# evenrose/CMDIAD

Measured on NVIDIA B200. Metric: patch-NN scores/sec at 200k x 768 bank, higher is better.
Workload: dtype f32 (fp16 tensor-core pre-filter with an error-bound certificate, exact fp32 re-check, FP32-equivalent fp16 hi/lo fallback)

## Files before the change

cmdiad_b200/csrc/score_gemm.cu:

```cuda
#include <cuda.h>

#include <cstdlib>

#include "common.cuh"

namespace cmdb {

constexpr int BM = kScoreBM;
constexpr int BN = kScoreBN;
constexpr int BK = kScoreBK;
constexpr int UMMA_K = 16;
constexpr int kGemmCtlThreads = 128;
constexpr uint32_t kTileABytes = BM * BK * 2;
constexpr uint32_t kTileBBytes = BN * BK * 2;
constexpr uint32_t kTmemCols = 512;

template <int TERMS, int CG>
struct GemmSmem {
    static constexpr uint32_t kTileB = kTileBBytes / CG;
    static constexpr int kStages = (TERMS == 3 ? 2 : 4) * (CG == 2 ? 3 : 2) / 2;
    static constexpr uint32_t kStageBytes = (TERMS == 3 ? 2u : 1u) * (kTileABytes + kTileB);
    static constexpr uint32_t stage(int s) { return s * kStageBytes; }
    static constexpr uint32_t a_hi(int s) { return stage(s); }
    static constexpr uint32_t b_hi(int s) { return stage(s) + kTileABytes; }
// ... 101 lines not shown
__device__ __forceinline__ void tc_fence_before() { asm volatile("tcgen05.fence::before_thread_sync;" ::: "memory"); }
__device__ __forceinline__ void tc_fence_after() { asm volatile("tcgen05.fence::after_thread_sync;" ::: "memory"); }
__device__ __forceinline__ void tmem_ld32(uint32_t taddr, uint32_t (&r)[32]) {
    asm volatile(
        "tcgen05.ld.sync.aligned.32x32b.x32.b32 "
        "{%0,%1,%2,%3,%4,%5,%6,%7,%8,%9,%10,%11,%12,%13,%14,%15,%16,%17,%18,%19,%20,%21,%22,%23,%24,%25,%26,%27,%28,%29,%30,%31}, "
        "[%32];"
        : "=r"(r[0]), "=r"(r[1]), "=r"(r[2]), "=r"(r[3]), "=r"(r[4]), "=r"(r[5]), "=r"(r[6]), "=r"(r[7]), "=r"(r[8]),
          "=r"(r[9]), "=r"(r[10]), "=r"(r[11]), "=r"(r[12]), "=r"(r[13]), "=r"(r[14]), "=r"(r[15]), "=r"(r[16]),
          "=r"(r[17]), "=r"(r[18]), "=r"(r[19]), "=r"(r[20]), "=r"(r[21]), "=r"(r[22]), "=r"(r[23]), "=r"(r[24]),
          "=r"(r[25]), "=r"(r[26]), "=r"(r[27]), "=r"(r[28]), "=r"(r[29]), "=r"(r[30]), "=r"(r[31])
        : "r"(taddr)
        : "memory");
}
__device__ __forceinline__ void tmem_ld_wait() { asm volatile("tcgen05.wait::ld.sync.aligned;" ::: "memory"); }

__device__ __forceinline__ uint64_t make_sw128_desc(uint32_t smem_addr) {
    uint64_t d = 0;
    d |= (uint64_t)((smem_addr & 0x3FFFFu) >> 4);
    d |= (uint64_t)((8u * BK * 2u) >> 4) << 32;
    d |= (uint64_t)1 << 46;
    d |= (uint64_t)2 << 61;
    return d;
}
constexpr uint32_t kIdesc = (1u << 4) | ((uint32_t)(BN >> 3) << 17) | ((uint32_t)(BM >> 4) << 24);
constexpr uint32_t kIdescPair = (1u << 4) | ((uint32_t)(BN >> 3) << 17) | ((uint32_t)((2 * BM) >> 4) << 24);

__device__ __forceinline__ int tile_stride(int mt, int G) {
    for (int s = mt;; ++s) {
        int a = s % G, b = G;
        if (a == 0) a = G;
        while (b) {
            const int t = a % b;
            a = b, b = t;
        }
        if (a == 1 || G == 1) return s;
    }
}
struct TileIter {
    int n, m, base, smod, G;
    __device__ __forceinline__ TileIter(int c, int G_, int mt, int stride) {
        G = G_;
        smod = stride % G;
        n = -1, m = mt, base = (c + smod) % G;
    }
    __device__ __forceinline__ bool next(int mt, int nt) {
        m += G;
        while (m >= mt) {
            if (++n >= nt) return false;
            base -= smod;
            if (base < 0) base += G;
            m = base;
        }
        return true;
    }
};

struct Top2 {
    float b1, b2;
    int i1, i2;
};
__device__ __forceinline__ void top2_update(Top2 &t, float v, int col) {
    const bool c1 = v < t.b1, c2 = v < t.b2;
    t.i2 = c1 ? t.i1 : (c2 ? col : t.i2);
    t.b2 = fminf(t.b2, fmaxf(t.b1, v));
    t.i1 = c1 ? col : t.i1;
    t.b1 = fminf(t.b1, v);
}
__device__ __forceinline__ void top2_insert(Top2 &t, float v, int i) {
    if (i < 0) return;
    const bool c1 = t.i1 < 0 || v < t.b1 || (v == t.b1 && i < t.i1);
    const bool c2 = t.i2 < 0 || v < t.b2 || (v == t.b2 && i < t.i2);
    if (c1) t.b2 = t.b1, t.i2 = t.i1, t.b1 = v, t.i1 = i;
    else if (c2) t.b2 = v, t.i2 = i;
}
__device__ __forceinline__ void top2_chunk(const uint32_t (&r)[32], float c, const float *bn, int col, Top2 &ta, Top2 &tb) {
#pragma unroll
    for (int k = 0; k < 32; k += 2) {
        top2_update(ta, fmaf(__uint_as_float(r[k]), c, bn[k]), col + k);
        top2_update(tb, fmaf(__uint_as_float(r[k + 1]), c, bn[k + 1]), col + k + 1);
    }
}

struct GemmParams {
    int mt;
    int m_base;
    const int *m_count;
    int nt;
    int kb;
    const float *bnorm;
    const int *q_scale_exp;
    int b_scale_exp;
    float4 *cand;
    int cand_stride;
    int run;
};

template <int TERMS, int EG, int CG>
__global__ void __launch_bounds__(kGemmCtlThreads + 128 * EG, 1)
score_gemm_kernel(const __grid_constant__ CUtensorMap tm_qhi, const __grid_constant__ CUtensorMap tm_qlo,
                  const __grid_constant__ CUtensorMap tm_bhi, const __grid_constant__ CUtensorMap tm_blo, GemmParams p) {
    using S = GemmSmem<TERMS, CG>;
    constexpr int kGemmThreads = kGemmCtlThreads + 128 * EG;
    extern __shared__ __align__(1024) unsigned char smem_raw[];
    unsigned char *smem = smem_raw + ((1024u - (smem_u32(smem_raw) & 1023u)) & 1023u);
    const uint32_t sbase = smem_u32(smem);
    const int warp = threadIdx.x >> 5, lane = threadIdx.x & 31;
    if (p.m_count) {
        p.mt = (__ldg(p.m_count) + BM - 1) / BM;
        if (p.mt == 0) return;
    }
    const int rank = CG == 2 ? (int)cluster_ctarank() : 0;
    const int unit = (int)blockIdx.x / CG, n_units = (int)gridDim.x / CG;
    const int mt_units = (p.mt + CG - 1) / CG;
    const int stride = tile_stride(mt_units, n_units);
    const int nruns = (p.nt + p.run - 1) / p.run;
    const uint32_t bar_full = sbase + S::bars, bar_empty = bar_full + 8 * S::kStages;
    const uint32_t bar_tfull = bar_empty + 8 * S::kStages, bar_tempty = bar_tfull + 16;
    uint32_t *tmem_slot = reinterpret_cast<uint32_t *>(smem + S::bars + 8 * (2 * S::kStages + 4));
    float *bnorm_s = reinterpret_cast<float *>(smem + S::bnorm);
    float4 *state = p.cand + (size_t)blockIdx.x * EG * p.cand_stride;

    if (warp == 1 && lane == 0) {
        for (int s = 0; s < S::kStages; ++s) {
            mbar_init(bar_full + 8 * s, 1);
            mbar_init(bar_empty + 8 * s, 1);
        }
        for (int b = 0; b < 2; ++b) {
            mbar_init(bar_tfull + 8 * b, 1);
            mbar_init(bar_tempty + 8 * b, 4 * EG * CG);
        }
        asm volatile("fence.mbarrier_init.release.cluster;" ::: "memory");
    }
    if (warp == 2) {
        if constexpr (CG == 2) tmem_alloc_pair(smem_u32(tmem_slot), kTmemCols);
        else tmem_alloc(smem_u32(tmem_slot), kTmemCols);
    }
    for (int i = p.m_base * BM + threadIdx.x; i < (p.m_base + p.mt) * BM; i += kGemmThreads)
#pragma unroll
        for (int g = 0; g < EG; ++g)
            state[(size_t)g * p.cand_stride + i] = make_float4(INFINITY, __int_as_float(-1), INFINITY, __int_as_float(-1));
    __threadfence_block();
    tc_fence_before();
    __syncthreads();
    if constexpr (CG == 2) cluster_sync_all();
    tc_fence_after();
    const uint32_t tmem_base = *tmem_slot;

    if (warp == 0) {
        if (lane == 0) {
            int stage = 0;
            uint32_t phase = 0;
            for (TileIter it(unit, n_units, mt_units, stride); it.next(mt_units, nruns);) {
              const int m = it.m * CG + rank;
              for (int n = it.n * p.run, n_end = min(p.nt, n + p.run); n < n_end; ++n) {
                const int a_row = (p.m_base + m) * BM, b_row = n * BN + rank * (BN / CG);
                for (int kb = 0; kb < p.kb; ++kb) {
                    mbar_wait(bar_empty + 8 * stage, phase ^ 1);
                    if constexpr (CG == 2) {
                        const uint32_t full = map_to_cta(bar_full + 8 * stage, 0);
                        if (rank == 0) mbar_expect_tx(bar_full + 8 * stage, 2 * S::kStageBytes);
                        tma_load_2d_pair(sbase + S::a_hi(stage), &tm_qhi, full, kb * BK, a_row);
                        tma_load_2d_pair(sbase + S::b_hi(stage), &tm_bhi, full, kb * BK, b_row);
                        if constexpr (TERMS == 3) {
                            tma_load_2d_pair(sbase + S::a_lo(stage), &tm_qlo, full, kb * BK, a_row);
                            tma_load_2d_pair(sbase + S::b_lo(stage), &tm_blo, full, kb * BK, b_row);
                        }
                    } else {
                        const uint32_t full = bar_full + 8 * stage;
                        mbar_expect_tx(full, S::kStageBytes);
                        tma_load_2d(sbase + S::a_hi(stage), &tm_qhi, full, kb * BK, a_row);
                        tma_load_2d(sbase + S::b_hi(stage), &tm_bhi, full, kb * BK, b_row);
                        if constexpr (TERMS == 3) {
                            tma_load_2d(sbase + S::a_lo(stage), &tm_qlo, full, kb * BK, a_row);
                            tma_load_2d(sbase + S::b_lo(stage), &tm_blo, full, kb * BK, b_row);
                        }
                    }
                    if (++stage == S::kStages) stage = 0, phase ^= 1;
                }
              }
            }
        }
    } else if (warp == 1) {
        if (lane == 0 && rank == 0) {
            int stage = 0;
            uint32_t phase = 0;
            int j = 0;
            for (TileIter it(unit, n_units, mt_units, stride); it.next(mt_units, nruns);)
              for (int n = it.n * p.run, n_end = min(p.nt, n + p.run); n < n_end; ++n, ++j) {
                const int buf = j & 1;
                mbar_wait(bar_tempty + 8 * buf, ((j >> 1) & 1) ^ 1);
                tc_fence_after();
                const uint32_t tmem_d = tmem_base + buf * BN;
                for (int kb = 0; kb < p.kb; ++kb) {
                    mbar_wait(bar_full + 8 * stage, phase);
                    tc_fence_after();
                    const uint64_t a_hi = make_sw128_desc(sbase + S::a_hi(stage));
                    const uint64_t a_lo = make_sw128_desc(sbase + S::a_lo(stage));
                    const uint64_t b_hi = make_sw128_desc(sbase + S::b_hi(stage));
                    const uint64_t b_lo = make_sw128_desc(sbase + S::b_lo(stage));
#pragma unroll
                    for (int ks = 0; ks < BK / UMMA_K; ++ks) {
                        const uint64_t adv = (uint64_t)((ks * UMMA_K * 2) >> 4);
                        if constexpr (CG == 2) {
                            umma_f16_pair(tmem_d, a_hi + adv, b_hi + adv, kIdescPair, (kb | ks) != 0);
                            if constexpr (TERMS == 3) {
                                umma_f16_pair(tmem_d, a_hi + adv, b_lo + adv, kIdescPair, 1);
                                umma_f16_pair(tmem_d, a_lo + adv, b_hi + adv, kIdescPair, 1);
                            }
                        } else {
                            umma_f16(tmem_d, a_hi + adv, b_hi + adv, kIdesc, (kb | ks) != 0);
                            if constexpr (TERMS == 3) {
                                umma_f16(tmem_d, a_hi + adv, b_lo + adv, kIdesc, 1);
                                umma_f16(tmem_d, a_lo + adv, b_hi + adv, kIdesc, 1);
                            }
                        }
                    }
                    if constexpr (CG == 2) umma_commit_pair(bar_empty + 8 * stage);
                    else umma_commit(bar_empty + 8 * stage);
                    if (++stage == S::kStages) stage = 0, phase ^= 1;
                }
                if constexpr (CG == 2) umma_commit_pair(bar_tfull + 8 * buf);
                else umma_commit(bar_tfull + 8 * buf);
            }
        }
    } else if (warp >= 4) {
        const int quarter = warp & 3;
        const int half = (warp - 4) >> 2;
        const int row = quarter * 32 + lane;
        const int et = threadIdx.x - kGemmCtlThreads;
        constexpr int kHalfCols = BN / EG;
        float4 *my_state = state + (size_t)half * p.cand_stride;
        const uint32_t tempty_leader = CG == 2 ? map_to_cta(bar_tempty, 0) : bar_tempty;
        auto release_tmem = [&](int buf) {
            tc_fence_before();
            __syncwarp();
            if (lane == 0) {
                if constexpr (CG == 2) mbar_arrive_cluster(tempty_leader + 8 * buf);
                else mbar_arrive(bar_tempty + 8 * buf);
            }
        };
        int j = 0;
        for (TileIter it(unit, n_units, mt_units, stride); it.next(mt_units, nruns);) {
          const int m_tile = it.m * CG + rank;
          const bool valid = m_tile < p.mt;
          const int m_local = p.m_base + m_tile;
          float c = 0.f;
          Top2 ta{INFINITY, INFINITY, -1, -1};
          if (valid) {
              c = ldexpf(-2.f, -(p.b_scale_exp + __ldg(p.q_scale_exp + m_local * BM + row)));
              const float4 st = my_state[m_local * BM + row];
              ta = Top2{st.x, st.z, __float_as_int(st.y), __float_as_int(st.w)};
          }
          for (int n = it.n * p.run, n_end = min(p.nt, n + p.run); n < n_end; ++n, ++j) {
            const int buf = j & 1;
            float *bn = bnorm_s + buf * BN;
#pragma unroll
            for (int g = 0; g < 2 / EG; ++g) bn[et + g * 128 * EG] = __ldg(p.bnorm + (size_t)n * BN + et + g * 128 * EG);
            Top2 tb{INFINITY, INFINITY, -1, -1};
            mbar_wait(bar_tfull + 8 * buf, (j >> 1) & 1);
            tc_fence_after();
            asm volatile("bar.sync 1, %0;" ::"n"(128 * EG) : "memory");
            if (!valid) {
                release_tmem(buf);
                continue;
            }
            const uint32_t taddr = tmem_base + ((uint32_t)(quarter * 32) << 16) + buf * BN + half * kHalfCols;
            const int col0 = n * BN + half * kHalfCols;
            const float *bnh = bn + half * kHalfCols;
            uint32_t ra[32], rb[32];
            tmem_ld32(taddr, ra);
#pragma unroll 1
            for (int ch = 0; ch < kHalfCols / 32; ch += 2) {
                tmem_ld_wait();
                tmem_ld32(taddr + (ch + 1) * 32, rb);
                top2_chunk(ra, c, bnh + ch * 32, col0 + ch * 32, ta, tb);
                tmem_ld_wait();
                if (ch + 2 < kHalfCols / 32) tmem_ld32(taddr + (ch + 2) * 32, ra);
                else release_tmem(buf);
                top2_chunk(rb, c, bnh + (ch + 1) * 32, col0 + (ch + 1) * 32, ta, tb);
            }
            top2_insert(ta, tb.b1, tb.i1);
            top2_insert(ta, tb.b2, tb.i2);
          }
          if (valid) my_state[m_local * BM + row] = make_float4(ta.b1, __int_as_float(ta.i1), ta.b2, __int_as_float(ta.i2));
        }
    }
    tc_fence_before();
    __syncthreads();
    if constexpr (CG == 2) cluster_sync_all();
    if (warp == 2) {
        tc_fence_after();
        if constexpr (CG == 2) tmem_dealloc_pair(tmem_base, kTmemCols);
        else tmem_dealloc(tmem_base, kTmemCols);
    }
}

__global__ void __launch_bounds__(256) q_split_kernel(const float *__restrict__ q, int P, int P_pad, int dim,
                                                      __half *__restrict__ hi, __half *__restrict__ lo,
                                                      int *__restrict__ scale_exp_out, float *__restrict__ q_norm,
                                                      float *__restrict__ q_eps, const int *__restrict__ list,
                                                      const int *__restrict__ count) {
    const int lane = threadIdx.x & 31, dim4 = dim >> 2;
    if (count) {
        P = __ldg(count);
        P_pad = (P + BM - 1) / BM * BM;
    }
    for (int r = blockIdx.x * 8 + (threadIdx.x >> 5); r < P_pad; r += gridDim.x * 8) {
        uint2 *h = reinterpret_cast<uint2 *>(hi + (size_t)r * dim), *l = reinterpret_cast<uint2 *>(lo + (size_t)r * dim);
        const float *src = q + (size_t)((list && r < P) ? __ldg(list + r) : r) * dim;
        float amax = 0.f;
        if (r < P)
            for (int cc = lane; cc < dim4; cc += 32) {
                const float4 v = __ldg(reinterpret_cast<const float4 *>(src) + cc);
                amax = fmaxf(fmaxf(amax, fmaxf(fabsf(v.x), fabsf(v.y))), fmaxf(fabsf(v.z), fabsf(v.w)));
            }
#pragma unroll
        for (int o = 16; o > 0; o >>= 1) amax = fmaxf(amax, __shfl_xor_sync(0xffffffffu, amax, o));
        int e = 0;
        if (amax > 0.f && amax < INFINITY) {
            int ex;
            frexpf(amax, &ex);
            e = 13 - ex;
        }
        if (lane == 0) scale_exp_out[r] = e;
        const float scale = ldexpf(1.f, e);
        float n2 = 0.f, e2 = 0.f;
        for (int cc = lane; cc < dim4; cc += 32) {
            float4 v = make_float4(0.f, 0.f, 0.f, 0.f);
            if (r < P) v = __ldg(reinterpret_cast<const float4 *>(src) + cc);
            v.x *= scale, v.y *= scale, v.z *= scale, v.w *= scale;
            __half2 h0 = __floats2half2_rn(v.x, v.y), h1 = __floats2half2_rn(v.z, v.w);
            const float2 f0 = __half22float2(h0), f1 = __half22float2(h1);
            const float r0 = v.x - f0.x, r1 = v.y - f0.y, r2 = v.z - f1.x, r3 = v.w - f1.y;
            n2 = fmaf(v.x, v.x, fmaf(v.y, v.y, fmaf(v.z, v.z, fmaf(v.w, v.w, n2))));
            e2 = fmaf(r0, r0, fmaf(r1, r1, fmaf(r2, r2, fmaf(r3, r3, e2))));
            __half2 l0 = __floats2half2_rn(r0, r1), l1 = __floats2half2_rn(r2, r3);
            h[cc] = make_uint2(*reinterpret_cast<unsigned int *>(&h0), *reinterpret_cast<unsigned int *>(&h1));
            l[cc] = make_uint2(*reinterpret_cast<unsigned int *>(&l0), *reinterpret_cast<unsigned int *>(&l1));
        }
        if (q_norm) {
#pragma unroll
            for (int o = 16; o > 0; o >>= 1) {
                n2 += __shfl_xor_sync(0xffffffffu, n2, o);
                e2 += __shfl_xor_sync(0xffffffffu, e2, o);
            }
            if (lane == 0) {
                const float inv = ldexpf(1.f, -e);
                q_norm[r] = __fmul_ru(__fsqrt_ru(n2), inv) * 1.001f;
                q_eps[r] = __fmul_ru(__fsqrt_ru(e2), inv) * 1.001f;
            }
        }
    }
}

typedef CUresult (*EncodeTiledFn)(CUtensorMap *, CUtensorMapDataType, cuuint32_t, void *, const cuuint64_t *, const cuuint64_t *,
                                  const cuuint32_t *, const cuuint32_t *, CUtensorMapInterleave, CUtensorMapSwizzle,
                                  CUtensorMapL2promotion, CUtensorMapFloatOOBfill);

static EncodeTiledFn get_encode_fn() {
    static EncodeTiledFn fn = nullptr;
    if (!fn) {
        void *p = nullptr;
        cudaDriverEntryPointQueryResult q;
        if (cudaGetDriverEntryPoint("cuTensorMapEncodeTiled", &p, cudaEnableDefault, &q) == cudaSuccess &&
            q == cudaDriverEntryPointSuccess)
            fn = reinterpret_cast<EncodeTiledFn>(p);
// ... 236 lines not shown
```

cmdiad_b200/csrc/score_tail.cu:

```cuda
#include <math.h>

#include "common.cuh"

namespace cmdb {

__device__ __forceinline__ unsigned long long pack_min_key(float v, unsigned int idx) {
    return ((unsigned long long)__float_as_uint(v) << 32) | idx;
}

__device__ __forceinline__ float warp_sqdist(const float *__restrict__ a, const float *__restrict__ b, int dim4, int lane) {
    float acc = 0.f;
    for (int c = lane; c < dim4; c += 32) {
        const float4 x = __ldg(reinterpret_cast<const float4 *>(a) + c), y = __ldg(reinterpret_cast<const float4 *>(b) + c);
        float d;
        d = x.x - y.x, acc = fmaf(d, d, acc);
        d = x.y - y.y, acc = fmaf(d, d, acc);
        d = x.z - y.z, acc = fmaf(d, d, acc);
        d = x.w - y.w, acc = fmaf(d, d, acc);
    }
#pragma unroll
    for (int o = 16; o > 0; o >>= 1) acc += __shfl_xor_sync(0xffffffffu, acc, o);
    return acc;
}

// ... 36 lines not shown
    if (qc >= (count ? __ldg(count) : P)) return;
    const int qi = list ? __ldg(list + qc) : qc;
    float tv[kRefineTop];
    int ti[kRefineTop];
#pragma unroll
    for (int k = 0; k < kRefineTop; ++k) tv[k] = INFINITY, ti[k] = -1;
    auto insert = [&](float v, int i) {
        if (i < 0) return;
#pragma unroll
        for (int k = 0; k < kRefineTop; ++k) {
            if (ti[k] == i) return;
            if (v < tv[k] || (v == tv[k] && i < ti[k]) || ti[k] < 0) {
                float fv = tv[k];
                int fi = ti[k];
                tv[k] = v, ti[k] = i;
                v = fv, i = fi;
                if (i < 0) return;
            }
        }
    };
    for (int c = lane; c < n_cand; c += 32) {
        const float4 t = cand[(size_t)c * cand_stride + qc];
        insert(t.x, __float_as_int(t.y));
        insert(t.z, __float_as_int(t.w));
    }
    int sel_idx[kRefineTop];
#pragma unroll
    for (int r = 0; r < kRefineTop; ++r) {
        float v = tv[0];
        int i = ti[0];
        if (i < 0) v = INFINITY;
#pragma unroll
        for (int o = 16; o > 0; o >>= 1) {
            const float ov = __shfl_xor_sync(0xffffffffu, v, o);
            const int oi = __shfl_xor_sync(0xffffffffu, i, o);
            if (oi >= 0 && (i < 0 || ov < v || (ov == v && oi < i))) v = ov, i = oi;
        }
        sel_idx[r] = i;
        if (i >= 0 && ti[0] == i) {
#pragma unroll
            for (int k = 0; k + 1 < kRefineTop; ++k) tv[k] = tv[k + 1], ti[k] = ti[k + 1];
            tv[kRefineTop - 1] = INFINITY, ti[kRefineTop - 1] = -1;
        }
    }
    float best = INFINITY;
    int best_i = -1;
#pragma unroll
    for (int r = 0; r < kRefineTop; ++r) {
        const int i = sel_idx[r];
        if (i < 0) continue;
        const float d2 = warp_sqdist(q + (size_t)qi * dim, bank + (size_t)i * dim, dim >> 2, lane);
        if (best_i < 0 || d2 < best || (d2 == best && i < best_i)) best = d2, best_i = i;
    }
    if (lane == 0) {
        const float dv = sqrtf(best);
        min_val[qi] = dv;
        min_idx[qi] = best_i < 0 ? -1 : (long long)best_i + row_offset;
        atomicMax(s_key + qi / P_img,
                  ((unsigned long long)__float_as_uint(dv) << 32) | (0xffffffffu - (unsigned int)(qi % P_img)));
    }
}

constexpr int kCertThreads = 256;
constexpr int kCertRows = 24;

__device__ __forceinline__ void cert_recheck(const int *list, int n_list, const float *__restrict__ qrow, const float *__restrict__ bank,
                                             int dim, int lane, float &best, int &best_i) {
    const int dim4 = dim >> 2;
    for (int j = 0; j < n_list; j += 4) {
        const int r0 = list[j], r1 = list[min(j + 1, n_list - 1)], r2 = list[min(j + 2, n_list - 1)], r3 = list[min(j + 3, n_list - 1)];
        float d[4];
        if (j + 1 < n_list) {
            warp_sqdist4(qrow, bank + (size_t)r0 * dim, bank + (size_t)r1 * dim, bank + (size_t)r2 * dim, bank + (size_t)r3 * dim,
                         dim4, lane, d);
        } else {
            d[0] = warp_sqdist(qrow, bank + (size_t)r0 * dim, dim4, lane);
            d[1] = d[2] = d[3] = d[0];
        }
        const int rr[4] = {r0, r1, r2, r3};
#pragma unroll
        for (int k = 0; k < 4; ++k)
            if (best_i < 0 || d[k] < best || (d[k] == best && rr[k] < best_i)) best = d[k], best_i = rr[k];
    }
}

template <int QB>
__global__ void __launch_bounds__(kCertThreads) refine_cert_kernel(const float4 *__restrict__ cand, int n_cand, int cand_stride,
                                                          const float *__restrict__ q, const float *__restrict__ bank, int dim,
                                                          int P, int P_img, long long row_offset,
                                                          const float *__restrict__ q_norm, const float *__restrict__ q_eps,
                                                          float bmax, float eb_max, float acc_model,
                                                          float *__restrict__ min_val,
                                                          long long *__restrict__ min_idx, unsigned long long *s_key,
                                                          int *__restrict__ fail_list, int *__restrict__ ctl,
                                                          int2 *__restrict__ work_list, unsigned long long *__restrict__ best_key) {
    constexpr int kWarps = kCertThreads / 32;
    constexpr int PL = 32 / QB;
    constexpr int CSTEP = kWarps * PL;
    __shared__ float part_s[CSTEP][QB];
    __shared__ float thr_s[QB];
    __shared__ int cnt_s[QB], bad_s[QB], list_s[QB][kCertRows];
    const int lane = threadIdx.x & 31, warp = threadIdx.x >> 5;
    const int ql = lane % QB;
    const int q0 = blockIdx.x * QB, qi = q0 + ql;
    const int cls = warp * PL + lane / QB;
    const bool live = qi < P;
    const float4 *col = cand + (live ? qi : q0);
    if (threadIdx.x < QB) cnt_s[threadIdx.x] = 0, bad_s[threadIdx.x] = 0;
    constexpr int kHold = QB <= 16 ? 320 / CSTEP : 8;
    const float4 empty = make_float4(INFINITY, __int_as_float(-1), INFINITY, __int_as_float(-1));
    float4 held[kHold];
    float v1 = INFINITY;
#pragma unroll
    for (int k = 0; k < kHold; ++k) {
        const int c = cls + k * CSTEP;
        held[k] = c < n_cand ? col[(size_t)c * cand_stride] : empty;
    }
#pragma unroll
    for (int k = 0; k < kHold; ++k)
        if (__float_as_int(held[k].y) >= 0) v1 = fminf(v1, held[k].x);
#pragma unroll 4
    for (int c = cls + kHold * CSTEP; c < n_cand; c += CSTEP) {
        const float4 t = col[(size_t)c * cand_stride];
        if (__float_as_int(t.y) >= 0) v1 = fminf(v1, t.x);
    }
    part_s[cls][ql] = v1;
    __syncthreads();
    if (threadIdx.x < QB) {
        float v1min = part_s[0][threadIdx.x];
#pragma unroll
        for (int k = 1; k < CSTEP; ++k) v1min = fminf(v1min, part_s[k][threadIdx.x]);
        const int qq = q0 + threadIdx.x;
        float thr = INFINITY;
        if (qq < P) {
            const float qn = q_norm[qq], qe = q_eps[qq];
            const float bh = __fadd_ru(bmax, eb_max);
            float E = __fmul_ru(qe, bh);
            E = __fmaf_ru(qn, eb_max, E);
            E = __fmaf_ru(__fmul_ru(acc_model, __fadd_ru(qn, qe)), bh, E);
            E = __fmul_ru(2.f, E);
            const float span = __fadd_ru(qn, bmax);
            E = __fmaf_ru(__fmul_ru((float)(dim + 16) * 5.9604645e-8f, span), span, E);
            const float t = __fadd_ru(v1min, __fmul_ru(2.0625f, E));
            if (v1min < INFINITY && t < INFINITY) thr = t;
        }
        thr_s[threadIdx.x] = thr;
    }
    __syncthreads();
    {
        const float thr = thr_s[ql];
        const bool all_in = !(thr < INFINITY);
        auto band = [&](const float4 t, int c) {
            const int i1 = __float_as_int(t.y), i2 = __float_as_int(t.w);
            const bool in1 = i1 >= 0 && (t.x <= thr || all_in), in2 = i2 >= 0 && (t.z <= thr || all_in);
            bool queue = in2;
            if (in1) {
                const int slot = atomicAdd(&cnt_s[ql], 1);
                if (slot < kCertRows) list_s[ql][slot] = i1;
                else queue = true;
            }
            if (in2) {
                const int slot = atomicAdd(&cnt_s[ql], 1);
                if (slot < kCertRows) list_s[ql][slot] = i2;
            }
            if (queue) {
                atomicAdd(&bad_s[ql], 1);
                const int slot = atomicAdd(ctl + 1, 1);
                if (slot < kWorkCap) work_list[slot] = make_int2(qi, c);
            }
        };
        if (live) {
#pragma unroll
            for (int k = 0; k < kHold; ++k) band(held[k], cls + k * CSTEP);
#pragma unroll 4
            for (int c = cls + kHold * CSTEP; c < n_cand; c += CSTEP) band(col[(size_t)c * cand_stride], c);
        }
    }
    __syncthreads();
    for (int k = warp; k < QB; k += kWarps) {
        const int qq = q0 + k;
        if (qq >= P) break;
        float best = INFINITY;
        int best_i = -1;
        cert_recheck(list_s[k], min(cnt_s[k], kCertRows), q + (size_t)qq * dim, bank, dim, lane, best, best_i);
        if (lane == 0) {
            if (bad_s[k] == 0 && best_i >= 0) {
                const float dv = sqrtf(best);
                min_val[qq] = dv;
                min_idx[qq] = (long long)best_i + row_offset;
                atomicMax(s_key + qq / P_img,
                          ((unsigned long long)__float_as_uint(dv) << 32) | (0xffffffffu - (unsigned int)(qq % P_img)));
            } else {
                fail_list[atomicAdd(ctl + 0, 1)] = qq;
                best_key[qq] = best_i < 0 ? ~0ULL : (((unsigned long long)__float_as_uint(best) << 32) | (unsigned int)best_i);
            }
        }
    }
    __syncthreads();
    if (threadIdx.x == 0) {
        __threadfence();
        if (atomicAdd(ctl + 5, 1) == (int)gridDim.x - 1) {
            __threadfence();
            const int fails = atomicAdd(ctl + 0, 0), pairs = atomicAdd(ctl + 1, 0);
            const bool rescan = fallback_use_rescan(fails, pairs);
            ctl[2] = rescan ? 0 : fails;
            ctl[3] = rescan ? pairs : 0;
            ctl[4] = rescan ? fails : 0;
        }
    }
}

__device__ __forceinline__ int producer_first_tile(int c, int m, int G, int stride) {
    const int want = ((c - m % G) % G + G) % G, smod = stride % G;
    int n0 = 0;
    for (int x = 0; x != want; ++n0) {
        x += smod;
        if (x >= G) x -= G;
    }
    return n0;
}

__global__ void __launch_bounds__(256) rescan_kernel(const int2 *__restrict__ work, const int *__restrict__ n_items_ptr,
                                                     const float *__restrict__ q, const float *__restrict__ bank, int dim,
                                                     long long rows, int n_units, int cg, int EG, int nt, int chunk_tiles,
                                                     int mt_total, int inv_full, int inv_last, int run_full,
// ... 490 lines not shown
        const unsigned long long *src = p.block_keys + (size_t)b * gridDim.x * 3;
        for (int i = lane; i < (int)gridDim.x * 3; i += 32) top3_insert(t, __ldcg(src + i));
        warp_top3(t, f);
        const unsigned long long skey = p.s_key[b];
        const float s_star = __uint_as_float((unsigned int)(skey >> 32));
        const int s_idx = s_idx_sh[b];
        float knn[2] = {NAN, NAN};
#pragma unroll
        for (int k = 0; k < 2; ++k)
            if (f[1 + k] != ~0ULL)
                knn[k] = sqrtf(warp_sqdist(p.q + ((size_t)b * p.P_img + s_idx) * dim,
                                           p.bank + (size_t)((long long)(f[1 + k] & 0xffffffffULL) - p.row_offset) * dim,
                                           dim4, lane));
        if (lane == 0) {
            TailResult *res = p.res + b;
            p.top3[b * 3 + 0] = f[0], p.top3[b * 3 + 1] = f[1], p.top3[b * 3 + 2] = f[2];
            res->s_idx = s_idx;
            res->s_star = s_star;
            res->m_star_row = g_sh[b];
            for (int k = 0; k < 3; ++k) res->nn_idx[k] = f[k] == ~0ULL ? -1 : (long long)(f[k] & 0xffffffffULL);
            const float Dn = sqrtf((float)dim);
            const float den = expf(knn[0] / Dn) + expf(knn[1] / Dn);
            const float w = 1.f - expf(s_star / Dn) / den;
            res->w = w;
            res->s = w * s_star;
            res->knn0 = knn[0], res->knn1 = knn[1];
        }
    }
}

struct ReweightCertParams {
    const float4 *cand;
    int n_cand, cand_stride;
    const float *m_star;
    const float *m_test;
    const float *bank;
    long long rows, row_offset;
    int dim;
    const float *q_norm, *q_eps;
    float bmax, eb_max, acc_model;
    int n_units, cg, EG, stride, nt, run;
    const unsigned long long *s_key;
    unsigned long long *top3;
    TailResult *res;
    int fuse_final;
};

__device__ __forceinline__ unsigned int float_order_bits(float v) {
    const unsigned int b = __float_as_uint(v);
    return b ^ ((b >> 31) ? 0xffffffffu : 0x80000000u);
}
__device__ __forceinline__ float float_from_order_bits(unsigned int u) {
    return __uint_as_float(u ^ ((u >> 31) ? 0x80000000u : 0xffffffffu));
}

__global__ void __launch_bounds__(256) reweight_cert_kernel(ReweightCertParams p) {
    constexpr int kMaxProd = 2 * 160;
    __shared__ unsigned long long wkeys[8][3];
    __shared__ int cand_rows[kMaxProd];
    __shared__ int bad_prod[kMaxProd];
    __shared__ int n_rows_sh, n_bad_sh;
    __shared__ float thr_sh;
    const int b = blockIdx.x, lane = threadIdx.x & 31, warp = threadIdx.x >> 5;
    const int dim = p.dim, dim4 = dim >> 2;
    const float *ms = p.m_star + (size_t)b * dim;
    if (threadIdx.x == 0) n_rows_sh = 0, n_bad_sh = 0;
    unsigned long long t3[3] = {~0ULL, ~0ULL, ~0ULL}, f3[3];
    for (int c = threadIdx.x; c < p.n_cand; c += blockDim.x) {
        const float4 t = p.cand[(size_t)c * p.cand_stride + b];
        const int i1 = __float_as_int(t.y), i2 = __float_as_int(t.w);
        if (i1 >= 0) top3_insert(t3, ((unsigned long long)float_order_bits(t.x) << 32) | (unsigned int)i1);
        if (i2 >= 0) top3_insert(t3, ((unsigned long long)float_order_bits(t.z) << 32) | (unsigned int)i2);
    }
    warp_top3(t3, f3);
    if (lane == 0) wkeys[warp][0] = f3[0], wkeys[warp][1] = f3[1], wkeys[warp][2] = f3[2];
    __syncthreads();
    if (threadIdx.x == 0) {
        unsigned long long g3[3] = {~0ULL, ~0ULL, ~0ULL};
        for (int w = 0; w < 8; ++w)
            for (int k = 0; k < 3; ++k) top3_insert(g3, wkeys[w][k]);
        float thr = INFINITY;
        if (g3[2] != ~0ULL) {
            const float v3 = float_from_order_bits((unsigned int)(g3[2] >> 32));
            const float qn = p.q_norm[b], qe = p.q_eps[b];
            const float bh = __fadd_ru(p.bmax, p.eb_max);
            float E = __fmul_ru(qe, bh);
            E = __fmaf_ru(qn, p.eb_max, E);
            E = __fmaf_ru(__fmul_ru(p.acc_model, __fadd_ru(qn, qe)), bh, E);
            E = __fmul_ru(2.f, E);
            const float span = __fadd_ru(qn, p.bmax);
            E = __fmaf_ru(__fmul_ru((float)(dim + 16) * 5.9604645e-8f, span), span, E);
            thr = __fadd_ru(v3, __fmul_ru(2.0625f, E));
            if (!(thr == thr)) thr = INFINITY;
        }
        thr_sh = thr;
    }
    __syncthreads();
    const float thr = thr_sh;
    for (int c = threadIdx.x; c < p.n_cand; c += blockDim.x) {
        const float4 t = p.cand[(size_t)c * p.cand_stride + b];
        const int i1 = __float_as_int(t.y), i2 = __float_as_int(t.w);
        if (i2 >= 0 && !(t.z > thr)) bad_prod[atomicAdd(&n_bad_sh, 1)] = c;
        else if (i1 >= 0 && !(t.x > thr)) cand_rows[atomicAdd(&n_rows_sh, 1)] = i1;
    }
    __syncthreads();
    unsigned long long w3[3] = {~0ULL, ~0ULL, ~0ULL};
    auto visit = [&](long long r) {
        const float d2 = warp_sqdist(ms, p.bank + (size_t)r * dim, dim4, lane);
        const unsigned long long key = pack_min_key(d2, (unsigned int)(r + p.row_offset));
        if (key != w3[0] && key != w3[1] && key != w3[2]) top3_insert(w3, key);
    };
    const int n_rows = n_rows_sh, n_bad = n_bad_sh;
    for (int i = warp; i < n_rows; i += 8) visit(cand_rows[i]);
    const int cols = kScoreBN / p.EG;
    const int nruns = (p.nt + p.run - 1) / p.run, runs_per = (nruns + p.n_units - 1) / p.n_units;
    for (int i = 0; i < n_bad; ++i) {
        const int c = bad_prod[i] / p.EG, g = bad_prod[i] % p.EG;
        const int j0 = producer_first_tile(c / p.cg, (b / kScoreBM) / p.cg, p.n_units, p.stride);
        for (int j = warp; j < runs_per * p.run * cols; j += 8) {
            const int k = j / (p.run * cols), t = (j / cols) % p.run;
            const int jrun = j0 + k * p.n_units;
            const int n = jrun * p.run + t;
            const long long r = (long long)n * kScoreBN + g * cols + j % cols;
            if (jrun < nruns && n < p.nt && r < p.rows) visit(r);
        }
    }
    if (lane == 0) wkeys[warp][0] = w3[0], wkeys[warp][1] = w3[1], wkeys[warp][2] = w3[2];
    __syncthreads();
    if (warp != 0) return;
    unsigned long long f[3] = {~0ULL, ~0ULL, ~0ULL};
    for (int w = 0; w < 8; ++w)
        for (int k = 0; k < 3; ++k) {
            const unsigned long long key = wkeys[w][k];
            if (key != f[0] && key != f[1] && key != f[2]) top3_insert(f, key);
        }
    float s_star = 0.f;
    float knn[2] = {NAN, NAN};
    if (p.fuse_final) {
        s_star = __uint_as_float((unsigned int)(p.s_key[b] >> 32));
#pragma unroll
        for (int k = 0; k < 2; ++k)
            if (f[1 + k] != ~0ULL)
                knn[k] = sqrtf(warp_sqdist(p.m_test + (size_t)b * dim,
                                           p.bank + (size_t)((long long)(f[1 + k] & 0xffffffffULL) - p.row_offset) * dim, dim4, lane));
    }
    if (lane == 0) {
        p.top3[(size_t)b * 3 + 0] = f[0], p.top3[(size_t)b * 3 + 1] = f[1], p.top3[(size_t)b * 3 + 2] = f[2];
        if (!p.res) return;
        TailResult *res = p.res + b;
        for (int k = 0; k < 3; ++k) res->nn_idx[k] = f[k] == ~0ULL ? -1 : (long long)(f[k] & 0xffffffffULL);
        if (p.fuse_final) {
            const float Dn = sqrtf((float)dim);
            const float den = expf(knn[0] / Dn) + expf(knn[1] / Dn);
            const float w = 1.f - expf(s_star / Dn) / den;
            res->w = w;
            res->s = w * s_star;
            res->knn0 = knn[0], res->knn1 = knn[1];
        }
    }
}

__global__ void __launch_bounds__(64) reweight_lookup_kernel(const unsigned long long *__restrict__ table, const float *__restrict__ m_test,
                                                            const float *__restrict__ bank, int dim,
                                                            const unsigned long long *__restrict__ s_key, unsigned long long *top3,
                                                            TailResult *res_all) {
    const int b = blockIdx.x, lane = threadIdx.x & 31, warp = threadIdx.x >> 5;
    __shared__ float knn[2];
    TailResult *res = res_all + b;
    const unsigned long long *keys3 = table + (size_t)res->m_star_row * 3;
    const unsigned long long key = keys3[1 + warp];
    float v = NAN;
    if (key != ~0ULL) v = sqrtf(warp_sqdist(m_test + (size_t)b * dim, bank + (size_t)(key & 0xffffffffULL) * dim, dim >> 2, lane));
    if (lane == 0) knn[warp] = v;
    __syncthreads();
// ... 496 lines not shown
```

Measured before the change: 4.182 million.

## Pack column index into score low bits for branchless top-2 in fp16 epilogue

For the single-term fp16 pre-filter GEMM, the epilogue now stores the within-chunk column index in the low 5 mantissa bits of each score. Each 32-column chunk is then reduced with min/max instructions instead of index-tracking compare-and-select, and the row index is rebuilt afterwards. The perturbation this adds to the scores is covered by an extra term in the certificate error bound, so the exact re-check stays valid. Candidate-state initialisation and the state reload are also skipped when each CTA covers the full N range, which saves global memory traffic.

```diff
diff --git a/cmdiad_b200/csrc/score_gemm.cu b/cmdiad_b200/csrc/score_gemm.cu
--- a/cmdiad_b200/csrc/score_gemm.cu
+++ b/cmdiad_b200/csrc/score_gemm.cu
@@ -207,6 +207,45 @@
     }
 }
 
+constexpr int kKeyBits = 5;
+__device__ __forceinline__ float pack_key(float v, int k, uint32_t mask) {
+    uint32_t d;
+    asm("lop3.b32 %0, %1, %2, %3, 0xEC;" : "=r"(d) : "r"(__float_as_uint(v)), "r"(k), "r"(mask));
+    return __uint_as_float(d);
+}
+__device__ __forceinline__ int key_row(float key, int chunk_row) {
+    return key < INFINITY ? chunk_row | (__float_as_int(key) & ((1 << kKeyBits) - 1)) : -1;
+}
+__device__ __forceinline__ float fmin3(float a, float b, float c) {
+    float d;
+    asm("min.f32 %0, %1, %2, %3;" : "=f"(d) : "f"(a), "f"(b), "f"(c));
+    return d;
+}
+__device__ __forceinline__ float fmax_nan(float a, float b) {
+    float d;
+    asm("max.NaN.f32 %0, %1, %2;" : "=f"(d) : "f"(a), "f"(b));
+    return d;
+}
+__device__ __forceinline__ void key_top2_chunk(const uint32_t (&r)[32], float c, const float *bn, int chunk_row, Top2 &t) {
+    const float o1 = t.b1, o2 = t.b2;
+    float b1 = o1, b2 = o2;
+    uint32_t mask;
+    asm("mov.b32 %0, %1;" : "=r"(mask) : "n"(~((1u << kKeyBits) - 1)));
+#pragma unroll
+    for (int k = 0; k < 32; k += 2) {
+        const float x = pack_key(fmaf(__uint_as_float(r[k]), c, bn[k]), k, mask);
+        const float y = pack_key(fmaf(__uint_as_float(r[k + 1]), c, bn[k + 1]), k + 1, mask);
+        const float lo = fminf(x, y), hi = fmax_nan(x, y);
+        b2 = fmin3(b2, hi, fmax_nan(b1, lo));
+        b1 = fminf(b1, lo);
+    }
+    const bool new1 = b1 != o1;
+    const bool held2 = b2 == (new1 ? o1 : o2);
+    t.i2 = held2 ? (new1 ? t.i1 : t.i2) : chunk_row;
+    t.i1 = new1 ? chunk_row : t.i1;
+    t.b1 = b1, t.b2 = b2;
+}
+
 struct GemmParams {
     int mt;
     int m_base;
@@ -261,10 +300,11 @@
         if constexpr (CG == 2) tmem_alloc_pair(smem_u32(tmem_slot), kTmemCols);
         else tmem_alloc(smem_u32(tmem_slot), kTmemCols);
     }
-    for (int i = p.m_base * BM + threadIdx.x; i < (p.m_base + p.mt) * BM; i += kGemmThreads)
+    if (CG == 2 || nruns < n_units)
+        for (int i = p.m_base * BM + threadIdx.x; i < (p.m_base + p.mt) * BM; i += kGemmThreads)
 #pragma unroll
-        for (int g = 0; g < EG; ++g)
-            state[(size_t)g * p.cand_stride + i] = make_float4(INFINITY, __int_as_float(-1), INFINITY, __int_as_float(-1));
+            for (int g = 0; g < EG; ++g)
+                state[(size_t)g * p.cand_stride + i] = make_float4(INFINITY, __int_as_float(-1), INFINITY, __int_as_float(-1));
     __threadfence_block();
     tc_fence_before();
     __syncthreads();
@@ -374,8 +414,11 @@
           Top2 ta{INFINITY, INFINITY, -1, -1};
           if (valid) {
               c = ldexpf(-2.f, -(p.b_scale_exp + __ldg(p.q_scale_exp + m_local * BM + row)));
+          }
+          if (valid && it.n >= n_units) {
               const float4 st = my_state[m_local * BM + row];
               ta = Top2{st.x, st.z, __float_as_int(st.y), __float_as_int(st.w)};
+              if constexpr (TERMS == 1) ta.i1 &= -32, ta.i2 &= -32;
           }
           for (int n = it.n * p.run, n_end = min(p.nt, n + p.run); n < n_end; ++n, ++j) {
             const int buf = j & 1;
@@ -393,21 +436,28 @@
             const uint32_t taddr = tmem_base + ((uint32_t)(quarter * 32) << 16) + buf * BN + half * kHalfCols;
             const int col0 = n * BN + half * kHalfCols;
             const float *bnh = bn + half * kHalfCols;
+            auto chunk = [&](const uint32_t(&r)[32], int ch) {
+                if constexpr (TERMS == 1) key_top2_chunk(r, c, bnh + ch * 32, col0 + ch * 32, ta);
+                else top2_chunk(r, c, bnh + ch * 32, col0 + ch * 32, ta, tb);
+            };
             uint32_t ra[32], rb[32];
             tmem_ld32(taddr, ra);
 #pragma unroll 1
             for (int ch = 0; ch < kHalfCols / 32; ch += 2) {
                 tmem_ld_wait();
                 tmem_ld32(taddr + (ch + 1) * 32, rb);
-                top2_chunk(ra, c, bnh + ch * 32, col0 + ch * 32, ta, tb);
+                chunk(ra, ch);
                 tmem_ld_wait();
                 if (ch + 2 < kHalfCols / 32) tmem_ld32(taddr + (ch + 2) * 32, ra);
                 else release_tmem(buf);
-                top2_chunk(rb, c, bnh + (ch + 1) * 32, col0 + (ch + 1) * 32, ta, tb);
-            }
-            top2_insert(ta, tb.b1, tb.i1);
-            top2_insert(ta, tb.b2, tb.i2);
+                chunk(rb, ch + 1);
+            }
+            if constexpr (TERMS == 3) {
+                top2_insert(ta, tb.b1, tb.i1);
+                top2_insert(ta, tb.b2, tb.i2);
+            }
           }
+          if constexpr (TERMS == 1) ta.i1 = key_row(ta.b1, ta.i1), ta.i2 = key_row(ta.b2, ta.i2);
           if (valid) my_state[m_local * BM + row] = make_float4(ta.b1, __int_as_float(ta.i1), ta.b2, __int_as_float(ta.i2));
         }
     }
diff --git a/cmdiad_b200/csrc/score_tail.cu b/cmdiad_b200/csrc/score_tail.cu
--- a/cmdiad_b200/csrc/score_tail.cu
+++ b/cmdiad_b200/csrc/score_tail.cu
@@ -142,6 +142,19 @@
         for (int k = 0; k < 4; ++k)
             if (best_i < 0 || d[k] < best || (d[k] == best && rr[k] < best_i)) best = d[k], best_i = rr[k];
     }
+}
+
+__device__ __forceinline__ float cert_error_bound(float qn, float qe, float bmax, float eb_max, float acc_model, int dim) {
+    const float bh = __fadd_ru(bmax, eb_max);
+    float E = __fmul_ru(qe, bh);
+    E = __fmaf_ru(qn, eb_max, E);
+    E = __fmaf_ru(__fmul_ru(acc_model, __fadd_ru(qn, qe)), bh, E);
+    E = __fmul_ru(2.f, E);
+    const float span = __fadd_ru(qn, bmax);
+    E = __fmaf_ru(__fmul_ru((float)(dim + 16) * 5.9604645e-8f, span), span, E);
+    const float V = __fmaf_ru(__fmul_ru(2.f, __fadd_ru(qn, qe)), bh, __fmul_ru(bh, bh));
+    E = __fmaf_ru(0x1p-18f, V, E);
+    return __fadd_ru(E, 0x1p-144f);
 }
 
 template <int QB>
@@ -193,14 +206,7 @@
         const int qq = q0 + threadIdx.x;
         float thr = INFINITY;
         if (qq < P) {
-            const float qn = q_norm[qq], qe = q_eps[qq];
-            const float bh = __fadd_ru(bmax, eb_max);
-            float E = __fmul_ru(qe, bh);
-            E = __fmaf_ru(qn, eb_max, E);
-            E = __fmaf_ru(__fmul_ru(acc_model, __fadd_ru(qn, qe)), bh, E);
-            E = __fmul_ru(2.f, E);
-            const float span = __fadd_ru(qn, bmax);
-            E = __fmaf_ru(__fmul_ru((float)(dim + 16) * 5.9604645e-8f, span), span, E);
+            const float E = cert_error_bound(q_norm[qq], q_eps[qq], bmax, eb_max, acc_model, dim);
             const float t = __fadd_ru(v1min, __fmul_ru(2.0625f, E));
             if (v1min < INFINITY && t < INFINITY) thr = t;
         }
@@ -857,14 +863,7 @@
         float thr = INFINITY;
         if (g3[2] != ~0ULL) {
             const float v3 = float_from_order_bits((unsigned int)(g3[2] >> 32));
-            const float qn = p.q_norm[b], qe = p.q_eps[b];
-            const float bh = __fadd_ru(p.bmax, p.eb_max);
-            float E = __fmul_ru(qe, bh);
-            E = __fmaf_ru(qn, p.eb_max, E);
-            E = __fmaf_ru(__fmul_ru(p.acc_model, __fadd_ru(qn, qe)), bh, E);
-            E = __fmul_ru(2.f, E);
-            const float span = __fadd_ru(qn, p.bmax);
-            E = __fmaf_ru(__fmul_ru((float)(dim + 16) * 5.9604645e-8f, span), span, E);
+            const float E = cert_error_bound(p.q_norm[b], p.q_eps[b], p.bmax, p.eb_max, p.acc_model, dim);
             thr = __fadd_ru(v3, __fmul_ru(2.0625f, E));
             if (!(thr == thr)) thr = INFINITY;
         }
```

Result: faster. 4.313 million, median of 6 (+3.1%).
